# zhenyuw16/Uni3DETR

Measured on AMD Instinct MI355X. Metric: scenes/sec (fwd+bwd) SUN-RGB-D 20k pts, 300 queries, higher is better.
Workload: dtype bf16

## Files before the change

### include/u3d_hip.h

```cpp
#ifndef U3D_HIP_H_
#define U3D_HIP_H_

#include <stddef.h>
#include <stdint.h>

#ifdef __cplusplus
extern "C" {
#endif

typedef struct ihipStream_t* u3d_stream;

enum {
  U3D_OK = 0,
  U3D_ERR_ARG = -1,
  U3D_ERR_UNSUPPORTED = -2,
  U3D_ERR_LAUNCH = -3,
  U3D_ERR_WORKSPACE = -4
};

enum { U3D_F32 = 0, U3D_BF16 = 1 };

int32_t u3d_version(void);
const char* u3d_strerror(int32_t code);

// ... 244 lines not shown
                     int32_t* out_count, int32_t* out_off, void* workspace, int64_t workspace_bytes, u3d_stream s);

#define U3D_DET_TAIL_SOFT_NMS 3
#define U3D_DET_TAIL_MERGE 4
int64_t u3d_det_tail_pp_workspace(int32_t batch, int32_t nq, int32_t num_classes, int32_t max_num, int32_t box_dim, int32_t mode);
int32_t u3d_det_tail_pp(const float* prob, const float* fused, const float* boxes, int32_t batch, int32_t nq, int32_t num_classes,
                        int32_t box_dim, int32_t max_num, const float* center_range, float score_threshold, int32_t mode, float nms_thr,
                        const float* score_thr, int32_t num_thr, float soft_sigma, float soft_prune, float* out_boxes, float* out_scores,
                        int32_t* out_labels, int32_t* out_count, int32_t* out_off, void* workspace, int64_t workspace_bytes, u3d_stream s);

int32_t u3d_tap_gather_sum(const void* p, const int32_t* nbr, int32_t ld, const int32_t* n_dev, int32_t n_cap, int32_t c,
                           int32_t kvol, int32_t dtype, void* out, u3d_stream s);
int32_t u3d_tap_gather_sum_add(const void* p, const int32_t* nbr, int32_t ld, const int32_t* n_dev, int32_t n_cap, int32_t c,
                               int32_t kvol, int32_t dtype, const void* addend, void* out, u3d_stream s);

int32_t u3d_layernorm_blocks(int32_t n);
int32_t u3d_layernorm_fwd(const void* x, int32_t x_dtype, int32_t n, int32_t c, const float* gamma, const float* beta,
                          float eps, int32_t relu, void* y, int32_t y_dtype, float* mean, float* rstd, u3d_stream s);
int32_t u3d_layernorm_bwd(const void* dy, int32_t y_dtype, const void* x, int32_t x_dtype, int32_t n, int32_t c,
                          const float* gamma, const float* beta, const float* mean, const float* rstd, int32_t relu,
                          void* dx, float* partial, u3d_stream s);

int64_t u3d_det_loss_workspace(int32_t L, int32_t m);
int32_t u3d_det_loss_fwd(const float* cls, const float* box, const float* iou_logit, const float* tgt, const int64_t* lab,
                         const float* w, const float* iou_true, const float* cls_avg, const float* npos, const float* code_w,
                         int32_t L, int32_t m, int32_t c, int32_t code, int32_t tdim, float alpha, float w_cls, float w_box,
                         float w_iou, float eps, float* out, void* workspace, int64_t workspace_bytes, u3d_stream s);
int32_t u3d_det_loss_bwd(const float* cls, const float* box, const float* iou_logit, const float* tgt, const int64_t* lab,
                         const float* w, const float* iou_true, const float* cls_avg, const float* npos, const float* code_w,
                         const float* gout, int32_t L, int32_t m, int32_t c, int32_t code, int32_t tdim, float alpha, float w_cls,
// ... 262 lines not shown
```

### uni3detr_amd/csrc/glds_epilogue.inc

```
  f32x4 cs[WN], cq[WN];
#pragma unroll
  for (int b = 0; b < WN; ++b) { cs[b] = (f32x4){0.f, 0.f, 0.f, 0.f}; cq[b] = (f32x4){0.f, 0.f, 0.f, 0.f}; }
#pragma unroll
  for (int a = 0; a < WM; ++a) {
    const int m = m0 + (wm * WM + a) * 16 + li;
    if (m >= n_out) continue;
#pragma unroll
    for (int b = 0; b < WN; ++b) {
      const int col = col0 + (wn * WN + b) * 16 + 4 * g;
      if (col < cout) {
        f32x4 v = acc[a][b];
        if (bias) {
          if (GLDS_EPI_ADDEND && (relu & 2)) {
            if constexpr (F32OUT) v += *(const f32x4*)(bias + (long long)m * cout + col);
            else v += __builtin_convertvector(*(const bf16x4*)((const u16*)bias + (long long)m * cout + col), f32x4);
          } else { const f32x4 bv = *(const f32x4*)(bias + col); v += bv; }
        }
        if (relu & 1) { v[0] = fmaxf(v[0], 0.f); v[1] = fmaxf(v[1], 0.f); v[2] = fmaxf(v[2], 0.f); v[3] = fmaxf(v[3], 0.f); }
        if constexpr (F32OUT) {
          *(f32x4*)((float*)out + (long long)m * cout + col) = v;
          if (stats) { cs[b] += v; cq[b] += v * v; }
          continue;
        }
        const bf16x4 o = __builtin_convertvector(v, bf16x4);
        *(bf16x4*)(out + (long long)m * cout + col) = o;
        if (stats) {
          const f32x4 vr = __builtin_convertvector(o, f32x4);
          if (GLDS_EPI_ADDEND && bn.x) {
            constexpr int CPR = BN / 8, SWZ = (CPR - 1) & 15;
            const int row = (wm * WM + a) * 16 + li, cc = (wn * WN + b) * 2 + (g >> 1);
            *(bf16x4*)(smem + ((row * CPR + (cc ^ (row & SWZ))) * 8 + (g & 1) * 4)) = o;
          } else {
            cs[b] += vr;
            cq[b] += vr * vr;
          }
        }
      }
    }
  }
  if (GLDS_EPI_ADDEND && stats && bn.x) {
// ... 13 lines not shown
          red[(wm * 2 + 0) * BN + cl] = s1;
          red[(wm * 2 + 1) * BN + cl] = s2;
        }
      }
    __syncthreads();
    for (int t = tid; t < 2 * BN; t += NW * 64) {
      const int which = t / BN, cl = t % BN;
      if (col0 + cl < cout) {
        double a = 0.0;
#pragma unroll
        for (int k = 0; k < WAVES_M; ++k) a += (double)red[(k * 2 + which) * BN + cl];
        stats[((long long)tile * 2 + which) * cout + col0 + cl] = a;
      }
    }
  }
```

### uni3detr_amd/csrc/igemm_bf16.hip

```cpp
#include "igemm_common.h"
#include "conv_in.h"
#include "igemm_direct.h"

struct BnEpi {
  const u16* x = nullptr;
  const u16* y = nullptr;
  const float *mean = nullptr, *invstd = nullptr, *gamma = nullptr, *beta = nullptr;
  int relu = 0, pad = 0;
};
template <int BM, int BN, int NT>
__device__ __forceinline__ void bn_bwd_tile_sums(const BnEpi bn, u16* smem, int m0, int col0, int n_out, int cout, int tile,
                                              double* __restrict__ stats, int tid) {
  constexpr int CPR = BN / 8, SWZ = (CPR - 1) & 15, R = NT / CPR, ROWS = BM / R, BATCH = ROWS < 8 ? ROWS : (ROWS % 8 == 0 ? 8 : (ROWS % 6 == 0 ? 6 : 4));
  static_assert(NT % CPR == 0 && BM % R == 0 && ROWS % BATCH == 0, "tile / thread mismatch");
  const int cc = tid % CPR, r0 = tid / CPR;
  const int col = col0 + cc * 8;
  const bool from_y = bn.relu && bn.y, remask = bn.relu && !bn.y;
  float s0[8], s1[8], mu[8], is[8], ga[8], be[8];
#pragma unroll
  for (int e = 0; e < 8; ++e) { s0[e] = 0.f; s1[e] = 0.f; mu[e] = 0.f; is[e] = 0.f; ga[e] = 0.f; be[e] = 0.f; }
  __syncthreads();
  if (col < cout) {
#pragma unroll
    for (int e = 0; e < 8; ++e) { mu[e] = bn.mean[col + e]; is[e] = bn.invstd[col + e]; }
// ... 239 lines not shown
template <int WAVES_M, int WAVES_N, int WM, int WN, bool WK, int BK = 64>
static int launch_igemm_fwd(const void* in, const void* w, const int32_t* nbr, int ld, void* out, const int32_t* n_out_dev,
                            int n_out_cap, int cin, int cout, int kvol, hipStream_t s, const float* bias = nullptr, int relu = 0) {
  constexpr int BM = WAVES_M * WM * 16, BN = WAVES_N * WN * 16;
  constexpr int LDA = BK + 8, LDW = WK ? BN + 16 : BK + 8;
  const size_t lds = 2 * (size_t)(BM * LDA + (WK ? BK * LDW : BN * LDW)) * 2;
  auto kern = k_igemm_fwd<WAVES_M, WAVES_N, WM, WN, WK, BK>;
  if (lds > 64 * 1024) U3D_ALLOW_LDS(kern, lds);
  dim3 grid(u3d_cdiv(n_out_cap, BM), u3d_cdiv(cout, BN));
  hipLaunchKernelGGL(kern, grid, dim3(WAVES_M * WAVES_N * 64), lds, s, (const u16*)in, (const u16*)w, nbr, ld, (u16*)out, n_out_dev,
                     n_out_cap, cin, cout, kvol, bias, relu);
  return hipGetLastError() == hipSuccess ? U3D_OK : U3D_ERR_LAUNCH;
}


template <int WAVES_M, int WAVES_N, int WM, int WN, bool F32OUT = false>
__device__ __forceinline__ void igemm_glds_body(const u16* __restrict__ in, const u16* __restrict__ w, const int* __restrict__ nbr,
                                                int ld, u16* __restrict__ out, const int* __restrict__ n_out_dev, int n_out_cap,
                                                int cin, int cout, int kvol, const float* __restrict__ bias, int relu,
                                                double* __restrict__ stats, const BnEpi bn) {
  constexpr int NW = WAVES_M * WAVES_N;
  constexpr int BM = WAVES_M * WM * 16, BN = WAVES_N * WN * 16, BK = 64;
  constexpr int A_ELEMS = BM * BK, W_ELEMS = BN * BK;
  constexpr int STAGE_ELEMS = A_ELEMS + W_ELEMS;
  constexpr int SEGS_A = BM / 8 / NW, SEGS_W = BN / 8 / NW;
  static_assert(BM % (8 * NW) == 0 && BN % (8 * NW) == 0, "tile/wave mismatch");
  extern __shared__ __attribute__((aligned(16))) u16 smem[];

  const int n_out = min(*n_out_dev, n_out_cap);
  const int tile = u3d_xcd_tile(blockIdx.x, (n_out + BM - 1) / BM);
  if (tile < 0) return;
  const int m0 = tile * BM;
  const int col0 = blockIdx.y * BN;
  const int tid = threadIdx.x, lane = tid & 63;
  const int wv = __builtin_amdgcn_readfirstlane(tid >> 6);
  const int wm = wv / WAVES_N, wn = wv % WAVES_N;
  const int kchunks = cin / BK;
  const int nstage = kvol * kchunks;

  f32x4 acc[WM][WN];
#pragma unroll
  for (int a = 0; a < WM; ++a)
#pragma unroll
    for (int b = 0; b < WN; ++b) acc[a][b] = (f32x4){0.f, 0.f, 0.f, 0.f};

  const __amdgpu_buffer_rsrc_t in_rs = __builtin_amdgcn_make_buffer_rsrc((void*)in, 0, -1, 0x00020000);
  const __amdgpu_buffer_rsrc_t w_rs = __builtin_amdgcn_make_buffer_rsrc((void*)w, 0, -1, 0x00020000);
  const unsigned row_bytes = (unsigned)cin * 2u;
  const int lrow = lane >> 3, lslot = lane & 7;
  unsigned a_part16[SEGS_A], w_voff[SEGS_W];
  int arow[SEGS_A];
#pragma unroll
  for (int u = 0; u < SEGS_A; ++u) {
    const int r = (wv * SEGS_A + u) * 8 + lrow;
    arow[u] = r;
    a_part16[u] = (unsigned)(lslot ^ ((r >> 1) & 7)) * 16u;
  }
#pragma unroll
  for (int u = 0; u < SEGS_W; ++u) {
    const int r = (wv * SEGS_W + u) * 8 + lrow;
    const int part = lslot ^ ((r >> 1) & 7);
    w_voff[u] = (col0 + r < cout) ? (unsigned)((col0 + r) * cin + part * 8) * 2u : 0xFFFFFFFFu;
  }
  int idx_cur[SEGS_A], idx_nxt[SEGS_A];
  auto load_idx_next = [&](int stage) {
    const int kap = stage % kvol;
#pragma unroll
    for (int u = 0; u < SEGS_A; ++u) {
      int m = m0 + arow[u];
      int mc = m < n_out ? m : n_out - 1;
      idx_nxt[u] = nbr ? nbr[(long long)kap * ld + mc] : mc;
    }
  };
  auto advance_idx = [&]() {
#pragma unroll
    for (int u = 0; u < SEGS_A; ++u) idx_cur[u] = (m0 + arow[u] < n_out) ? idx_nxt[u] : -1;
  };
  auto issue = [&](int st, int buf) {
    const int kap = st % kvol, c0 = (st / kvol) * BK;
    u16* Ab = smem + buf * STAGE_ELEMS + wv * (SEGS_A * 512);
    u16* Wb = smem + buf * STAGE_ELEMS + A_ELEMS + wv * (SEGS_W * 512);
    const unsigned a_soff = (unsigned)c0 * 2u;
    const unsigned w_soff = (unsigned)(kap * cin * cout + c0) * 2u;
#pragma unroll
    for (int u = 0; u < SEGS_A; ++u) {
      unsigned voff = idx_cur[u] >= 0 ? (unsigned)idx_cur[u] * row_bytes + a_part16[u] : 0xFFFFFFFFu;
      __builtin_amdgcn_raw_ptr_buffer_load_lds(in_rs, (lds_void_ptr)(Ab + u * 512), 16, voff, a_soff, 0, 0);
    }
#pragma unroll
    for (int u = 0; u < SEGS_W; ++u)
      __builtin_amdgcn_raw_ptr_buffer_load_lds(w_rs, (lds_void_ptr)(Wb + u * 512), 16, w_voff[u], w_soff, 0, 0);
  };
#if GLDS_FRAG_B128
  auto issue_one = [&](int st, int buf, int q) {
    const int kap = st % kvol, c0 = (st / kvol) * BK;
    if (q < SEGS_A) {
      u16* Ab = smem + buf * STAGE_ELEMS + wv * (SEGS_A * 512);
      unsigned voff = idx_cur[q] >= 0 ? (unsigned)idx_cur[q] * row_bytes + a_part16[q] : 0xFFFFFFFFu;
      __builtin_amdgcn_raw_ptr_buffer_load_lds(in_rs, (lds_void_ptr)(Ab + q * 512), 16, voff, (unsigned)c0 * 2u, 0, 0);
    } else {
      const int u = q - SEGS_A;
      u16* Wb = smem + buf * STAGE_ELEMS + A_ELEMS + wv * (SEGS_W * 512);
      __builtin_amdgcn_raw_ptr_buffer_load_lds(w_rs, (lds_void_ptr)(Wb + u * 512), 16, w_voff[u], (unsigned)(kap * cin * cout + c0) * 2u, 0, 0);
    }
  };
  const int g = lane >> 4, li = lane & 15, fsw = (lane >> 1) & 7;
  int foff[2];
#pragma unroll
  for (int ks = 0; ks < 2; ++ks) foff[ks] = ((ks * 4 + g) ^ fsw) << 3;
  typedef const volatile s16x8 __attribute__((address_space(3))) * lds_vptr;
// ... 5 lines not shown
  const int g = lane >> 4, li = lane & 15, fsw = (lane >> 1) & 7;
  int foff[2][2];
#pragma unroll
  for (int ks = 0; ks < 2; ++ks)
#pragma unroll
    for (int j = 0; j < 2; ++j) foff[ks][j] = (((ks * 4 + (g >> 1) + 2 * j) ^ fsw) << 3) + (g & 1) * 4;
  typedef const volatile s16x4 __attribute__((address_space(3))) * lds_vptr;
  auto frag = [&](const u16* rowp, int ks) {
    s16x4 x = *(lds_vptr)(rowp + foff[ks][0]);
    s16x4 y = *(lds_vptr)(rowp + foff[ks][1]);
    s16x8 v = {x[0], x[1], x[2], x[3], y[0], y[1], y[2], y[3]};
    return __builtin_bit_cast(bf16x8, v);
  };

#endif
  load_idx_next(0);
  advance_idx();
  load_idx_next(1 < nstage ? 1 : 0);
  issue(0, 0);
  __syncthreads();
  for (int st = 0; st < nstage; ++st) {
    const int buf = st & 1;
    const int nx = st + 1 < nstage ? st + 1 : st;
    advance_idx();
    load_idx_next(st + 2 < nstage ? st + 2 : nstage - 1);
#if !GLDS_DMA_SPREAD
    issue(nx, buf ^ 1);
#endif
    const u16* A = smem + buf * STAGE_ELEMS + (wm * WM * 16 + li) * BK;
    const u16* W = smem + buf * STAGE_ELEMS + A_ELEMS + (wn * WN * 16 + li) * BK;
#pragma unroll
    for (int ks = 0; ks < 2; ++ks) {
      bf16x8 af[WM];
#pragma unroll
      for (int a = 0; a < WM; ++a) af[a] = frag(A + a * 16 * BK, ks);
#pragma unroll
      for (int b = 0; b < WN; ++b) {
        bf16x8 bfr = frag(W + b * 16 * BK, ks);
#pragma unroll
        for (int a = 0; a < WM; ++a) acc[a][b] = __builtin_amdgcn_mfma_f32_16x16x32_bf16(bfr, af[a], acc[a][b], 0, 0, 0);
#if GLDS_DMA_SPREAD
        {
          constexpr int NQ = SEGS_A + SEGS_W, NG = (GLDS_DMA_SPREAD == 1) ? 2 * WN : (GLDS_DMA_SPREAD == 3 ? (WN > 1 ? WN / 2 : 1) : (GLDS_DMA_SPREAD == 4 ? WN + WN / 2 : WN));
          constexpr int PER = (NQ + NG - 1) / NG;
          const int grp = ks * WN + b;
          if (grp < NG) {
#pragma unroll
            for (int j = 0; j < PER; ++j)
              if (grp * PER + j < NQ) issue_one(nx, buf ^ 1, grp * PER + j);
          }
          __builtin_amdgcn_sched_barrier(0);
        }
#endif
      }
    }
    __syncthreads();
  }
#define GLDS_EPI_ADDEND (BM != 256 || BN != 256)
#include "glds_epilogue.inc"
#undef GLDS_EPI_ADDEND
}

#ifndef GLDS8_PRIO
#define GLDS8_PRIO 1
#endif
#ifndef GLDS8_BALANCE
#define GLDS8_BALANCE 1
#endif
#ifndef GLDS8_STAGGER
#define GLDS8_STAGGER 1
#endif
template <bool F32OUT = false, int RB = 4>
__device__ __forceinline__ void igemm_glds8_body(const u16* __restrict__ in, const u16* __restrict__ w, const int* __restrict__ nbr,
                                                 int ld, u16* __restrict__ out, const int* __restrict__ n_out_dev, int n_out_cap,
// ... 432 lines not shown
U3D_GLDS_KERNEL_X(k_igemm_glds_256x256, GLDS256_CFG)
U3D_GLDS_KERNEL(k_igemm_glds_256x128, 4, 2, 4, 4)
U3D_GLDS_KERNEL(k_igemm_glds_128x64, 4, 1, 2, 4)
U3D_GLDS_KERNEL(k_igemm_glds_128x128, 2, 2, 4, 4)
#undef U3D_GLDS_KERNEL
#define U3D_GLDS_KERNEL_F32O(NAME, A, B, C, D)                                                                                   \
  __global__ __launch_bounds__(A* B * 64) void NAME(const u16* in, const u16* w, const int* nbr, int ld, u16* out,               \
                                                    const int* n_out_dev, int n_out_cap, int cin, int cout, int kvol,            \
                                                    const float* bias, int relu, double* stats, BnEpi bn) {                      \
    igemm_glds_body<A, B, C, D, true>(in, w, nbr, ld, out, n_out_dev, n_out_cap, cin, cout, kvol, bias, relu, stats, bn);         \
  }
U3D_GLDS_KERNEL_F32O(k_igemm_glds_128x64_f32o, 4, 1, 2, 4)
U3D_GLDS_KERNEL_F32O(k_igemm_glds_128x128_f32o, 2, 2, 4, 4)
#undef U3D_GLDS_KERNEL_F32O
typedef void (*glds_kernel_t)(const u16*, const u16*, const int*, int, u16*, const int*, int, int, int, int, const float*, int, double*, BnEpi);


struct GldsKernel {
  glds_kernel_t bf16, f32;
  int rows, cols, threads;
  size_t lds;
  bool addend;
};
#define GLDS_GEOM(A, B, C, D) A * C * 16, B * D * 16, A * B * 64, (size_t)2 * (A * C * 16 + B * D * 16) * 64 * 2
#define GLDS_GEOM_X(...) GLDS_GEOM(__VA_ARGS__)
enum { G_256x256, G8_256x256, G8_192x256, G8_256x128, G8_192x128, G_256x128, G_128x128, G_128x64, G_COUNT };
static const GldsKernel GLDS_KERNELS[G_COUNT] = {
    {k_igemm_glds_256x256, nullptr, GLDS_GEOM_X(GLDS256_CFG), false},
    {k_igemm_glds8_256x256, k_igemm_glds8_256x256_f32o, 256, 256, 512, 2 * (256 + 256) * 64 * 2, true},
    {k_igemm_glds8_192x256, k_igemm_glds8_192x256_f32o, 192, 256, 512, 2 * (256 + 256) * 64 * 2, true},
// ... 141 lines not shown
}

extern "C" int32_t u3d_igemm_dgrad_bnstats_bf16(const void* in, const void* w, const int32_t* nbr, int32_t ld, const void* addend, void* out,
                                                const int32_t* n_out_dev, int32_t n_out_cap, int32_t cin, int32_t cout, int32_t kvol,
                                                const u3d_bn_epi* bn, double* stats, u3d_stream s) {
  U3D_REQUIRE(in && w && out && n_out_dev && nbr && bn && bn->x && bn->mean && bn->invstd && stats, U3D_ERR_ARG);
  U3D_REQUIRE(!bn->relu || bn->y || (bn->gamma && bn->beta), U3D_ERR_ARG);
  const FwdPlan p = fwd_plan(n_out_cap, cin, cout, kvol, true, true, EPI_BN_BWD);
  if (!p.served()) return U3D_ERR_UNSUPPORTED;
  BnEpi e;
  e.x = (const u16*)bn->x; e.y = (const u16*)bn->y; e.mean = bn->mean; e.invstd = bn->invstd; e.gamma = bn->gamma; e.beta = bn->beta;
  e.relu = bn->relu;
  return fwd_launch(p, in, w, nbr, ld, out, n_out_dev, n_out_cap, cin, cout, kvol, s, addend, addend ? 2 : 0, stats, e);
}

extern "C" int32_t u3d_igemm_fwd_bf16(const void* in, const void* w, const int32_t* nbr, int32_t ld, void* out,
                                      const int32_t* n_out_dev, int32_t n_out_cap, int32_t cin, int32_t cout, int32_t kvol,
                                      int32_t transpose_w, u3d_stream s) {
  U3D_REQUIRE(in && w && out && n_out_dev && (nbr || kvol == 1), U3D_ERR_ARG);
  if (!transpose_w && convin_shape(cin, cout, kvol))
    return u3d_launch_conv_in_fwd(in, w, nbr, ld, out, n_out_dev, n_out_cap, kvol, s);
  const FwdPlan p = fwd_plan(n_out_cap, cin, cout, kvol, nbr != nullptr, transpose_w != 0, EPI_PLAIN);
  if (p.served()) return fwd_launch(p, in, w, nbr, ld, out, n_out_dev, n_out_cap, cin, cout, kvol, s);
  if (n_out_cap > 0 && cin % 16 == 0 && cout % 16 == 0 && cin <= 64 && cout <= 64 && (cin < 64 || cout < 64)) {
#define IG_SMALL(WNV, BKV)                                                                                                                          \
    return transpose_w ? launch_igemm_fwd<4, 1, IGEMM_SMALL_WM, WNV, false, BKV>(in, w, nbr, ld, out, n_out_dev, n_out_cap, cin, cout, kvol, s)   \
                       : launch_igemm_fwd<4, 1, IGEMM_SMALL_WM, WNV, true, BKV>(in, w, nbr, ld, out, n_out_dev, n_out_cap, cin, cout, kvol, s);
    if (cin == 16 || cin == 32) {
      if (cout == 16) { IG_SMALL(1, 32) }
      if (cout == 32) { IG_SMALL(2, 32) }
// ... 17 lines not shown
```

### uni3detr_amd/native.py

```python
import ctypes as C
import os

import numpy as np
import torch

from . import abi

_HERE = os.path.dirname(os.path.abspath(__file__))
LIB_PATH = os.environ.get("U3D_LIB_PATH") or os.path.join(_HERE, "libu3d_hip.so")

_ABI = abi.load()
_K = _ABI.constants


def _struct(c_name, py_name):
    return abi.structure(_ABI.structs[c_name], py_name)


def _slot_names(prefix):
    names = sorted((v, n[len(prefix):]) for n, v in _K.items() if n.startswith(prefix))
    assert [v for v, _ in names] == list(range(len(names))) and names[-1][1] == "COUNT" and _K[prefix + "COUNT"] == len(names) - 1
    return [n for _, n in names[:-1]]


# ... 1343 lines not shown
    n = len(counts)
    assert n == len(caps) and n <= 8 and flag.dtype == torch.float32
    _check(lib().u3d_capacity_flag(_ptr_array(counts), (C.c_int32 * max(n, 1))(*[int(c) for c in caps]), n, _ptr(flag), _stream()),
           "capacity_flag")


def tap_gather_sum(p, nbr, n_dev, n, c, kvol, addend=None):
    out = torch.empty((n, c), dtype=p.dtype, device=p.device)
    if addend is not None:
        assert addend.shape == out.shape and addend.dtype == out.dtype and addend.is_contiguous()
    _check(lib().u3d_tap_gather_sum_add(_ptr(p), _ptr(nbr), nbr.shape[1], _ptr(n_dev), n, c, kvol, dtype_code(p), _ptr(addend), _ptr(out),
                                        _stream()), "tap_gather_sum")
    return out


def _ptr_array(tensors):
    arr = (C.c_void_p * len(tensors))()
    for i, t in enumerate(tensors):
        arr[i] = t.data_ptr()
    return arr


def _batch_chunks(outs, maxb):
    o, n = 0, len(outs)
    while o < n:
        e = min(n, o + maxb)
        while e < n and e > o + 1 and outs[e].data_ptr() == outs[e - 1].data_ptr():
            e -= 1
        if e < n and outs[e].data_ptr() == outs[e - 1].data_ptr():
            raise U3DError("a group of batch slots with one output is larger than the batch limit")
# ... 646 lines not shown
```

### uni3detr_amd/plugin/dense.py

```python

import numpy as np
import torch
from torch import nn

from .. import native as nv
from .. import sparse as sp
from ..registry import BACKBONES, NECKS


def _conv(cfg, cin, cout, kernel, stride=1, padding=0):
    cfg = dict(cfg)
    t = cfg.pop("type")
    if t != "Conv3d":
        raise NotImplementedError("the HIP dense path implements the Conv3d variant used by every shipped config")
    if cfg.get("bias", True):
        raise NotImplementedError("shipped configs build these convolutions with bias=False")
    return nn.Conv3d(cin, cout, kernel, stride=stride, padding=padding, **cfg)


def _norm(cfg, c):
    cfg = dict(cfg)
    t = cfg.pop("type")
    assert t == "BN3d", "shipped configs use BN3d"
    cfg.pop("requires_grad", None)
# ... 9 lines not shown
    _cache = {}

    @classmethod
    def conv(cls, device, batch, dims_in, ksize, stride, pad):
        key = ("c", str(device), batch, tuple(dims_in), tuple(ksize), tuple(stride), tuple(pad))
        g = cls._cache.get(key)
        if g is None:
            dims_out = tuple((d + 2 * p - k) // s + 1 for d, k, s, p in zip(dims_in, ksize, stride, pad))
            n_in = batch * dims_in[0] * dims_in[1] * dims_in[2]
            n_out = batch * dims_out[0] * dims_out[1] * dims_out[2]
            one = all(k == 1 for k in ksize) and all(s == 1 for s in stride)
            fwd = None if one else nv.dense_nbr_table(batch, dims_out, dims_in, ksize, stride, pad, 0, device)
            bwd = None if one else nv.dense_nbr_table(batch, dims_in, dims_out, ksize, stride, pad, 1, device)
            n_in_dev = torch.tensor([n_in], dtype=torch.int32, device=device)
            n_out_dev = torch.tensor([n_out], dtype=torch.int32, device=device)
            g = (sp.ConvGeom(fwd, bwd, n_in, n_in_dev, n_out, n_out_dev, kind="dense", strided=any(s > 1 for s in stride)), dims_out)
            cls._cache[key] = g
        return g

    @classmethod
    def upsample_index(cls, device, batch, dims_in, s):
        key = ("u", str(device), batch, tuple(dims_in), s)
        v = cls._cache.get(key)
        if v is None:
            D, H, W = dims_in
            b = torch.arange(batch, device=device).view(-1, 1, 1, 1)
            z = torch.arange(D, device=device).view(1, -1, 1, 1)
            y = torch.arange(H * s, device=device).view(1, 1, -1, 1)
            x = torch.arange(W * s, device=device).view(1, 1, 1, -1)
            in_row = ((b * D + z) * H + y // s) * W + x // s
            tap = (y % s) * s + (x % s)
# ... 175 lines not shown
```

### uni3detr_amd/sparse.py

```python
import collections
import contextlib
import os

import torch

from . import native as nv
from .shadow import conv_weights, halo_packs

K3, S1, P1 = (3, 3, 3), (1, 1, 1), (1, 1, 1)


class Level:

    def __init__(self, grid, coords, n, n_dev):
        self.grid, self.coords, self.n, self.n_dev = grid, coords, n, n_dev
        self.dims, self.batch = grid.dims, grid.batch
        self._subm = None
        self._halo = None

    def halo(self):
        if self._halo is None:
            h = nv.SubmHalo(self.subm_tables()[0], self.n_dev, self.n) if self.n <= nv.SubmHalo.MAX_ROWS else None
            self._halo = h if (h is not None and h.ok) else False
        return self._halo or None
# ... 31 lines not shown
    def __init__(self, n):
        self.n = self.remaining = n
        self.acc = None

    def step(self, din):
        self.remaining -= 1
        if self.remaining > 0:
            self.acc = din
            return None
        self.acc, self.remaining = None, self.n
        return din


class ConvGeom:

    def __init__(self, nbr_fwd, nbr_bwd, n_in, n_in_dev, n_out, n_out_dev, kind="sparse", strided=False):
        self.strided = strided
        self.nbr_fwd, self.nbr_bwd = nbr_fwd, nbr_bwd
        self.n_in, self.n_in_dev, self.n_out, self.n_out_dev = n_in, n_in_dev, n_out, n_out_dev
        self.kind = kind
        self.level = None


def level_from_coors(coors, batch, dims):
    dev = coors.device
    g = nv.BitGrid(batch, dims, dev)
    g.mark(coors)
    g.scan()
    n = coors.shape[0]
    g.set_row_capacity(n)
    rank = g.rank(coors)
    lvl = Level(g, g.coords(n), n, g.count_dev)
    return lvl, rank


def subm_geom(lvl):
# ... 2 lines not shown
    g.level = lvl
    return g


def strided_level(lvl, ksize, stride, pad, capacity=None):
    dims_out = tuple((d + 2 * p - k) // s + 1 for d, k, s, p in zip(lvl.dims, ksize, stride, pad))
    g = nv.BitGrid(lvl.batch, dims_out, lvl.coords.device)
    g.mark_strided(lvl.coords, lvl.n_dev, ksize, stride, pad)
    g.scan()
    n_out = int(g.count_dev.item()) if capacity is None else int(capacity)
    if capacity is not None:
        g.set_row_capacity(n_out)
    out = Level(g, g.coords(n_out), n_out, g.count_dev)
    fwd = lvl.grid.nbr_table(out.coords, out.n_dev, ksize, stride, pad, 0)
    bwd = g.nbr_table(lvl.coords, lvl.n_dev, ksize, stride, pad, 1)
    return out, ConvGeom(fwd, bwd, lvl.n, lvl.n_dev, n_out, out.n_dev, strided=True)


REV_SUBM_TABLE = True
SUBM_HALO = os.environ.get("U3D_SUBM_HALO", "1") == "1"
HALO_WGRAD = True
HALO_128 = True
STRIDED_DGRAD_SPLIT = True
NMAJOR_FWD = True
STRIDED_SPLIT_MIN_RATIO = 16
STRIDED_SPLIT_SPARSE_RATIO = 16


_CONV_USES = {}


def reset_conv_uses():
    _CONV_USES.clear()
    _PLANES_BWD.clear()


SPLIT_BF16 = os.environ.get("U3D_SPLIT_BF16", "1") == "1"
SPLIT_FUSED_ADD = True
# ... 71 lines not shown
            t = torch.arange(n_rows, dtype=torch.int32, device=geom.n_out_dev.device).view(1, -1)
        elif isinstance(t, nv.RevNbr):
            t = t.t.flip(0)
        lo = torch.where(t >= 0, t + plane, t)
        cache[key] = torch.cat([t, lo] if which == "wgrad" else [t, t, lo], 0).contiguous()
    return cache[key]


def _halo_of(geom, kvol, cin, cout):
    if not (SUBM_HALO and REV_SUBM_TABLE and geom.level is not None and kvol == 27 and cin == cout
            and (cin == 64 or (cin == 128 and HALO_128)) and geom.n_out >= 4096):
        return None
    return geom.level.halo()


_ConvRoute = collections.namedtuple("_ConvRoute", "split nmajor halo kvol cin cout strided_split")


def _conv_route(feats, kio_shape, geom):
    kvol, cin, cout = kio_shape[0] * kio_shape[1] * kio_shape[2], kio_shape[3], kio_shape[4]
    bf16 = feats.dtype == torch.bfloat16
    nmajor = NMAJOR_FWD and bf16 and ((cin % 64 == 0 and cout % 64 == 0) or nv.direct_serves(cin, cout, kvol))
    split = _split_serves(feats, cin, cout, kvol)
    if split == "narrow" and geom.nbr_fwd is None:
        split = None
    halo = _halo_of(geom, kvol, cin, cout) if (nmajor and not split) else None
    strided_split = bool(STRIDED_DGRAD_SPLIT and geom.strided and kvol > 1 and (bf16 or split == "wide") and cout % 64 == 0
                         and (kvol * cin) % 64 == 0
                         and geom.n_out * (STRIDED_SPLIT_SPARSE_RATIO if geom.kind == "sparse" else STRIDED_SPLIT_MIN_RATIO) <= geom.n_in)
    return _ConvRoute(split, nmajor, halo, kvol, cin, cout, strided_split)


def _pending_addend(ctx):
    tok, fan = ctx.res_token, ctx.fan_token
    dres = tok.dres if tok is not None else None
    facc = fan.acc if fan is not None else None
    if dres is not None and facc is not None:
        return dres + facc
    return facc if dres is None else dres


def _finish_din(ctx, din, taken):
    tok, fan = ctx.res_token, ctx.fan_token
    if din is not None and not taken:
        if fan is not None and fan.acc is not None:
# ... 100 lines not shown

def _input_grad(ctx, r, wc, dout):
    g, kvol, cin, cout = ctx.geom, r.kvol, r.cin, r.cout
    nbr = g.nbr_bwd if kvol > 1 else None
    add = _pending_addend(ctx)
    fits = add is not None and add.dtype == dout.dtype and add.is_contiguous() and tuple(add.shape) == (g.n_in, cin)
    if r.strided_split:
        prod = nv.linear_bf16(dout, wc.view(kvol * cin, cout), None, False)
        fan = ctx.fan_token
        if not (fits and fan is not None and add is fan.acc):
            add = None
        return nv.tap_gather_sum(prod, nbr, g.n_in_dev, g.n_in, cin, kvol, addend=add), add is not None
    bt = ctx.bn_in
    if bt is not None and (bt.c != cin or not (add is None or fits)):
        bt = None
    if r.halo is not None:
        if cin != 64:
            bt = None
        if not fits:
            add = None
        pk = ctx.pk_bwd if ctx.pk_bwd is not None else nv.subm_halo_wpack(wc)
        din = nv.subm_halo_conv(dout, pk, r.halo, krev=True, addend=add, want_stats=bt is not None, tag="spconv_dgrad",
                                bn_epi=None if bt is None else bt.epi)
        if bt is not None:
            din, st, tr = din
            bt.partial = (st, tr)
        return din, add is not None
    res = nv.spconv_dgrad_bnstats(dout, wc, nbr, g.n_in_dev, g.n_in, cin, add, bt.epi) if (bt is not None and kvol > 1) else None
    if res is not None:
        bt.partial = (res[1], res[2])
# ... 220 lines not shown
```

Before: 424.4.

## Add stride-class sorted dgrad for strided sparse convs with per-tile tap masks

New measurement: 426.6, median of 6. Within noise of the previous version (+0.5%).

```diff
diff --git a/include/u3d_hip.h b/include/u3d_hip.h
--- a/include/u3d_hip.h
+++ b/include/u3d_hip.h
@@ -282,6 +282,16 @@
 int32_t u3d_tap_gather_sum_add(const void* p, const int32_t* nbr, int32_t ld, const int32_t* n_dev, int32_t n_cap, int32_t c,
                                int32_t kvol, int32_t dtype, const void* addend, void* out, u3d_stream s);
 
+int64_t u3d_stride_sort_workspace(int32_t n_cap);
+int32_t u3d_stride_sort(const int32_t* nbr, int32_t ld, const int32_t* n_dev, int32_t n_cap, const int32_t* coors,
+                        const int32_t dims[3], const int32_t ksize[3], const int32_t stride[3], const int32_t pad[3],
+                        int32_t tile_rows, int32_t* order, int32_t* tbl, int32_t tbl_ld, int32_t* tile_mask, void* workspace,
+                        int64_t workspace_bytes, u3d_stream s);
+int32_t u3d_igemm_dgrad_sorted_plan(int32_t n_cap, int32_t cin, int32_t cout, int32_t kvol, int32_t* rows, int32_t* cols);
+int32_t u3d_igemm_dgrad_sorted_bf16(const void* in, const void* w, const int32_t* tbl, int32_t ld, const int32_t* tile_mask,
+                                    const int32_t* order, const void* addend, void* out, const int32_t* n_dev, int32_t n_cap,
+                                    int32_t cin, int32_t cout, int32_t kvol, u3d_stream s);
+
 int32_t u3d_layernorm_blocks(int32_t n);
 int32_t u3d_layernorm_fwd(const void* x, int32_t x_dtype, int32_t n, int32_t c, const float* gamma, const float* beta,
                           float eps, int32_t relu, void* y, int32_t y_dtype, float* mean, float* rstd, u3d_stream s);
diff --git a/uni3detr_amd/csrc/glds_epilogue.inc b/uni3detr_amd/csrc/glds_epilogue.inc
--- a/uni3detr_amd/csrc/glds_epilogue.inc
+++ b/uni3detr_amd/csrc/glds_epilogue.inc
@@ -1,3 +1,7 @@
+#ifndef GLDS_EPI_ROW
+#define GLDS_EPI_ROW(m) (m)
+#define GLDS_EPI_ROW_DEFAULTED
+#endif
   f32x4 cs[WN], cq[WN];
 #pragma unroll
   for (int b = 0; b < WN; ++b) { cs[b] = (f32x4){0.f, 0.f, 0.f, 0.f}; cq[b] = (f32x4){0.f, 0.f, 0.f, 0.f}; }
@@ -5,6 +9,7 @@
   for (int a = 0; a < WM; ++a) {
     const int m = m0 + (wm * WM + a) * 16 + li;
     if (m >= n_out) continue;
+    const int mo = GLDS_EPI_ROW(m);
 #pragma unroll
     for (int b = 0; b < WN; ++b) {
       const int col = col0 + (wn * WN + b) * 16 + 4 * g;
@@ -12,18 +17,18 @@
         f32x4 v = acc[a][b];
         if (bias) {
           if (GLDS_EPI_ADDEND && (relu & 2)) {
-            if constexpr (F32OUT) v += *(const f32x4*)(bias + (long long)m * cout + col);
-            else v += __builtin_convertvector(*(const bf16x4*)((const u16*)bias + (long long)m * cout + col), f32x4);
+            if constexpr (F32OUT) v += *(const f32x4*)(bias + (long long)mo * cout + col);
+            else v += __builtin_convertvector(*(const bf16x4*)((const u16*)bias + (long long)mo * cout + col), f32x4);
           } else { const f32x4 bv = *(const f32x4*)(bias + col); v += bv; }
         }
         if (relu & 1) { v[0] = fmaxf(v[0], 0.f); v[1] = fmaxf(v[1], 0.f); v[2] = fmaxf(v[2], 0.f); v[3] = fmaxf(v[3], 0.f); }
         if constexpr (F32OUT) {
-          *(f32x4*)((float*)out + (long long)m * cout + col) = v;
+          *(f32x4*)((float*)out + (long long)mo * cout + col) = v;
           if (stats) { cs[b] += v; cq[b] += v * v; }
           continue;
         }
         const bf16x4 o = __builtin_convertvector(v, bf16x4);
-        *(bf16x4*)(out + (long long)m * cout + col) = o;
+        *(bf16x4*)(out + (long long)mo * cout + col) = o;
         if (stats) {
           const f32x4 vr = __builtin_convertvector(o, f32x4);
           if (GLDS_EPI_ADDEND && bn.x) {
@@ -67,3 +72,7 @@
       }
     }
   }
+#ifdef GLDS_EPI_ROW_DEFAULTED
+#undef GLDS_EPI_ROW
+#undef GLDS_EPI_ROW_DEFAULTED
+#endif
diff --git a/uni3detr_amd/csrc/igemm_bf16.hip b/uni3detr_amd/csrc/igemm_bf16.hip
--- a/uni3detr_amd/csrc/igemm_bf16.hip
+++ b/uni3detr_amd/csrc/igemm_bf16.hip
@@ -277,11 +277,13 @@
 }
 
 
-template <int WAVES_M, int WAVES_N, int WM, int WN, bool F32OUT = false>
+template <int WAVES_M, int WAVES_N, int WM, int WN, bool F32OUT = false, bool SORTED = false>
 __device__ __forceinline__ void igemm_glds_body(const u16* __restrict__ in, const u16* __restrict__ w, const int* __restrict__ nbr,
                                                 int ld, u16* __restrict__ out, const int* __restrict__ n_out_dev, int n_out_cap,
                                                 int cin, int cout, int kvol, const float* __restrict__ bias, int relu,
-                                                double* __restrict__ stats, const BnEpi bn) {
+                                                double* __restrict__ stats, const BnEpi bn,
+                                                const unsigned* __restrict__ tile_mask = nullptr,
+                                                const int* __restrict__ out_rows = nullptr) {
   constexpr int NW = WAVES_M * WAVES_N;
   constexpr int BM = WAVES_M * WM * 16, BN = WAVES_N * WN * 16, BK = 64;
   constexpr int A_ELEMS = BM * BK, W_ELEMS = BN * BK;
@@ -299,7 +301,24 @@
   const int wv = __builtin_amdgcn_readfirstlane(tid >> 6);
   const int wm = wv / WAVES_N, wn = wv % WAVES_N;
   const int kchunks = cin / BK;
-  const int nstage = kvol * kchunks;
+  unsigned sw_mask = 0, sw_rem = 0;
+  int sw_c = 0, sw_left = 0;
+  if constexpr (SORTED) {
+    sw_mask = __builtin_amdgcn_readfirstlane(tile_mask[tile]) & (kvol >= 32 ? 0xFFFFFFFFu : ((1u << kvol) - 1u));
+    sw_rem = sw_mask;
+    sw_left = __builtin_popcount(sw_mask) * kchunks;
+  }
+  const int nstage = SORTED ? sw_left : kvol * kchunks;
+  int sw_k1 = 0, sw_c1 = 0, sw_k2 = 0, sw_c2 = 0;
+  auto sw_next = [&](int& kap, int& c0) {
+    if (sw_left > 0) {
+      kap = __builtin_ctz(sw_rem);
+      c0 = sw_c;
+      sw_rem &= sw_rem - 1u;
+      if (sw_rem == 0u) { sw_rem = sw_mask; sw_c += BK; }
+      --sw_left;
+    }
+  };
 
   f32x4 acc[WM][WN];
 #pragma unroll
@@ -327,7 +346,7 @@
   }
   int idx_cur[SEGS_A], idx_nxt[SEGS_A];
   auto load_idx_next = [&](int stage) {
-    const int kap = stage % kvol;
+    const int kap = SORTED ? stage : stage % kvol;
 #pragma unroll
     for (int u = 0; u < SEGS_A; ++u) {
       int m = m0 + arow[u];
@@ -340,7 +359,7 @@
     for (int u = 0; u < SEGS_A; ++u) idx_cur[u] = (m0 + arow[u] < n_out) ? idx_nxt[u] : -1;
   };
   auto issue = [&](int st, int buf) {
-    const int kap = st % kvol, c0 = (st / kvol) * BK;
+    const int kap = SORTED ? sw_k1 : st % kvol, c0 = SORTED ? sw_c1 : (st / kvol) * BK;
     u16* Ab = smem + buf * STAGE_ELEMS + wv * (SEGS_A * 512);
     u16* Wb = smem + buf * STAGE_ELEMS + A_ELEMS + wv * (SEGS_W * 512);
     const unsigned a_soff = (unsigned)c0 * 2u;
@@ -356,7 +375,7 @@
   };
 #if GLDS_FRAG_B128
   auto issue_one = [&](int st, int buf, int q) {
-    const int kap = st % kvol, c0 = (st / kvol) * BK;
+    const int kap = SORTED ? sw_k1 : st % kvol, c0 = SORTED ? sw_c1 : (st / kvol) * BK;
     if (q < SEGS_A) {
       u16* Ab = smem + buf * STAGE_ELEMS + wv * (SEGS_A * 512);
       unsigned voff = idx_cur[q] >= 0 ? (unsigned)idx_cur[q] * row_bytes + a_part16[q] : 0xFFFFFFFFu;
@@ -392,16 +411,29 @@
   };
 
 #endif
+  if (!SORTED || nstage > 0) {
+  if constexpr (SORTED) {
+    sw_next(sw_k1, sw_c1);
+    load_idx_next(sw_k1);
+    advance_idx();
+    sw_k2 = sw_k1; sw_c2 = sw_c1;
+    sw_next(sw_k2, sw_c2);
+    load_idx_next(sw_k2);
+    issue(0, 0);
+    sw_k1 = sw_k2; sw_c1 = sw_c2;
+    sw_next(sw_k2, sw_c2);
+  } else {
   load_idx_next(0);
   advance_idx();
   load_idx_next(1 < nstage ? 1 : 0);
   issue(0, 0);
+  }
   __syncthreads();
   for (int st = 0; st < nstage; ++st) {
     const int buf = st & 1;
     const int nx = st + 1 < nstage ? st + 1 : st;
     advance_idx();
-    load_idx_next(st + 2 < nstage ? st + 2 : nstage - 1);
+    load_idx_next(SORTED ? sw_k2 : (st + 2 < nstage ? st + 2 : nstage - 1));
 #if !GLDS_DMA_SPREAD
     issue(nx, buf ^ 1);
 #endif
@@ -432,10 +464,17 @@
 #endif
       }
     }
+    if constexpr (SORTED) {
+      sw_k1 = sw_k2; sw_c1 = sw_c2;
+      sw_next(sw_k2, sw_c2);
+    }
     __syncthreads();
   }
-#define GLDS_EPI_ADDEND (BM != 256 || BN != 256)
+  }
+#define GLDS_EPI_ADDEND (SORTED || BM != 256 || BN != 256)
+#define GLDS_EPI_ROW(m) (SORTED ? out_rows[m] : (m))
 #include "glds_epilogue.inc"
+#undef GLDS_EPI_ROW
 #undef GLDS_EPI_ADDEND
 }
 
@@ -898,6 +937,23 @@
 U3D_GLDS_KERNEL_F32O(k_igemm_glds_128x128_f32o, 2, 2, 4, 4)
 #undef U3D_GLDS_KERNEL_F32O
 typedef void (*glds_kernel_t)(const u16*, const u16*, const int*, int, u16*, const int*, int, int, int, int, const float*, int, double*, BnEpi);
+
+#define U3D_GLDS_SORTED_KERNEL(NAME, A, B, C, D)                                                                                 \
+  __global__ __launch_bounds__(A* B * 64) void NAME(const u16* in, const u16* w, const int* tbl, int ld, u16* out,               \
+                                                    const int* n_out_dev, int n_out_cap, int cin, int cout, int kvol,            \
+                                                    const float* addend, int relu, const unsigned* tile_mask,                    \
+                                                    const int* out_rows) {                                                       \
+    igemm_glds_body<A, B, C, D, false, true>(in, w, tbl, ld, out, n_out_dev, n_out_cap, cin, cout, kvol, addend, relu, nullptr,   \
+                                             BnEpi{}, tile_mask, out_rows);                                                      \
+  }
+U3D_GLDS_SORTED_KERNEL(k_igemm_glds_sorted_128x64, 4, 1, 2, 4)
+U3D_GLDS_SORTED_KERNEL(k_igemm_glds_sorted_128x128, 2, 2, 4, 4)
+#define U3D_GLDS_SORTED_KERNEL_X(NAME, ...) U3D_GLDS_SORTED_KERNEL(NAME, __VA_ARGS__)
+U3D_GLDS_SORTED_KERNEL_X(k_igemm_glds_sorted_256x256, GLDS256_CFG)
+#undef U3D_GLDS_SORTED_KERNEL_X
+#undef U3D_GLDS_SORTED_KERNEL
+typedef void (*glds_sorted_kernel_t)(const u16*, const u16*, const int*, int, u16*, const int*, int, int, int, int, const float*, int,
+                                     const unsigned*, const int*);
 
 
 struct GldsKernel {
@@ -1069,6 +1125,42 @@
   return fwd_launch(p, in, w, nbr, ld, out, n_out_dev, n_out_cap, cin, cout, kvol, s, addend, addend ? 2 : 0, stats, e);
 }
 
+struct SortedPlan {
+  glds_sorted_kernel_t fn = nullptr;
+  int rows = 0, cols = 0, threads = 0;
+  size_t lds = 0;
+};
+static SortedPlan sorted_plan(int n_cap, int cin, int cout, int kvol) {
+  SortedPlan p;
+  if (n_cap <= 0 || cin <= 0 || cout <= 0 || cin % 64 != 0 || cout % 64 != 0 || kvol < 1 || kvol > 27) return p;
+  if (cout % 256 == 0 && (long long)u3d_cdiv(n_cap, 256) * (cout / 256) >= 128) {
+    p.fn = k_igemm_glds_sorted_256x256; p.rows = 256; p.cols = 256; p.threads = 512;
+  } else if (cout % 128 == 0) { p.fn = k_igemm_glds_sorted_128x128; p.rows = 128; p.cols = 128; p.threads = 256; }
+  else { p.fn = k_igemm_glds_sorted_128x64; p.rows = 128; p.cols = 64; p.threads = 256; }
+  p.lds = (size_t)2 * (p.rows + p.cols) * 64 * 2;
+  return p;
+}
+extern "C" int32_t u3d_igemm_dgrad_sorted_plan(int32_t n_cap, int32_t cin, int32_t cout, int32_t kvol, int32_t* rows, int32_t* cols) {
+  U3D_REQUIRE(rows && cols, U3D_ERR_ARG);
+  const SortedPlan p = sorted_plan(n_cap, cin, cout, kvol);
+  if (!p.fn) return U3D_ERR_UNSUPPORTED;
+  *rows = p.rows;
+  *cols = p.cols;
+  return U3D_OK;
+}
+extern "C" int32_t u3d_igemm_dgrad_sorted_bf16(const void* in, const void* w, const int32_t* tbl, int32_t ld, const int32_t* tile_mask,
+                                               const int32_t* order, const void* addend, void* out, const int32_t* n_dev, int32_t n_cap,
+                                               int32_t cin, int32_t cout, int32_t kvol, u3d_stream s) {
+  U3D_REQUIRE(in && w && tbl && tile_mask && order && out && n_dev && ld >= n_cap, U3D_ERR_ARG);
+  const SortedPlan p = sorted_plan(n_cap, cin, cout, kvol);
+  if (!p.fn) return U3D_ERR_UNSUPPORTED;
+  if (p.lds > 64 * 1024) U3D_ALLOW_LDS(p.fn, p.lds);
+  hipLaunchKernelGGL(p.fn, dim3(u3d_cdiv(n_cap, p.rows), cout / p.cols), dim3(p.threads), p.lds, (hipStream_t)s, (const u16*)in,
+                     (const u16*)w, tbl, ld, (u16*)out, n_dev, n_cap, cin, cout, kvol, (const float*)addend, addend ? 2 : 0,
+                     (const unsigned*)tile_mask, order);
+  return hipGetLastError() == hipSuccess ? U3D_OK : U3D_ERR_LAUNCH;
+}
+
 extern "C" int32_t u3d_igemm_fwd_bf16(const void* in, const void* w, const int32_t* nbr, int32_t ld, void* out,
                                       const int32_t* n_out_dev, int32_t n_out_cap, int32_t cin, int32_t cout, int32_t kvol,
                                       int32_t transpose_w, u3d_stream s) {
diff --git a/uni3detr_amd/csrc/stride_sort.hip b/uni3detr_amd/csrc/stride_sort.hip
--- /dev/null
+++ b/uni3detr_amd/csrc/stride_sort.hip
@@ -0,0 +1,154 @@
+#include "common.h"
+
+#define SSORT_MAX_CLASSES 64
+#define SSORT_BLOCK 256
+
+struct SortGeom {
+  int dz, dy, dx;
+  int s[3], p[3];
+  int ncls;
+};
+
+__device__ __forceinline__ int ssort_class(const int4* __restrict__ coors, const SortGeom& g, int m) {
+  int z, y, x;
+  if (coors) {
+    const int4 c = coors[m];
+    z = c.y; y = c.z; x = c.w;
+  } else {
+    x = m % g.dx;
+    const int t = m / g.dx;
+    y = t % g.dy;
+    z = (t / g.dy) % g.dz;
+  }
+  const int cz = (z + g.p[0]) % g.s[0], cy = (y + g.p[1]) % g.s[1], cx = (x + g.p[2]) % g.s[2];
+  return (cz * g.s[1] + cy) * g.s[2] + cx;
+}
+
+__device__ __forceinline__ int ssort_rank(int cls, int ncls, int (*cnt)[SSORT_BLOCK / 64], int& wave_rank) {
+  const int lane = threadIdx.x & 63, wv = threadIdx.x >> 6;
+  const unsigned long long below = (1ull << lane) - 1ull;
+  wave_rank = 0;
+  for (int c = 0; c < ncls; ++c) {
+    const unsigned long long b = __ballot(cls == c);
+    if (cls == c) wave_rank = __popcll(b & below);
+    if (lane == 0) cnt[c][wv] = __popcll(b);
+  }
+  __syncthreads();
+  return cls;
+}
+
+__global__ __launch_bounds__(SSORT_BLOCK) void k_ssort_hist(const int4* __restrict__ coors, SortGeom g, const int* __restrict__ n_dev,
+                                                           int n_cap, int nblocks, int* __restrict__ hist) {
+  __shared__ int cnt[SSORT_MAX_CLASSES][SSORT_BLOCK / 64];
+  const int n = min(*n_dev, n_cap);
+  const int m = blockIdx.x * SSORT_BLOCK + threadIdx.x;
+  const int cls = m < n ? ssort_class(coors, g, m) : -1;
+  int wr;
+  ssort_rank(cls, g.ncls, cnt, wr);
+  if ((int)threadIdx.x < g.ncls) {
+    int t = 0;
+#pragma unroll
+    for (int w = 0; w < SSORT_BLOCK / 64; ++w) t += cnt[threadIdx.x][w];
+    hist[threadIdx.x * nblocks + blockIdx.x] = t;
+  }
+}
+
+__global__ __launch_bounds__(1024) void k_ssort_scan(int* __restrict__ h, int e) {
+  __shared__ int part[1024];
+  const int tid = threadIdx.x, per = (e + 1023) / 1024;
+  const int b0 = min(tid * per, e), b1 = min(b0 + per, e);
+  int sum = 0;
+  for (int i = b0; i < b1; ++i) sum += h[i];
+  part[tid] = sum;
+  __syncthreads();
+  for (int off = 1; off < 1024; off <<= 1) {
+    const int v = tid >= off ? part[tid - off] : 0;
+    __syncthreads();
+    part[tid] += v;
+    __syncthreads();
+  }
+  int run = tid ? part[tid - 1] : 0;
+  for (int i = b0; i < b1; ++i) {
+    const int v = h[i];
+    h[i] = run;
+    run += v;
+  }
+}
+
+__global__ __launch_bounds__(SSORT_BLOCK) void k_ssort_scatter(const int4* __restrict__ coors, SortGeom g, const int* __restrict__ n_dev,
+                                                              int n_cap, int nblocks, const int* __restrict__ offs,
+                                                              int* __restrict__ order, const int* __restrict__ nbr, int ld, int kvol,
+                                                              int* __restrict__ tbl, int tld) {
+  __shared__ int cnt[SSORT_MAX_CLASSES][SSORT_BLOCK / 64];
+  const int n = min(*n_dev, n_cap);
+  const int m = blockIdx.x * SSORT_BLOCK + threadIdx.x;
+  const int cls = m < n ? ssort_class(coors, g, m) : -1;
+  int wr;
+  ssort_rank(cls, g.ncls, cnt, wr);
+  if (cls < 0) return;
+  const int wv = threadIdx.x >> 6;
+  int p = offs[cls * nblocks + blockIdx.x] + wr;
+  for (int w = 0; w < wv; ++w) p += cnt[cls][w];
+  if (p < 0 || p >= n_cap) return;
+  order[p] = m;
+  for (int k = 0; k < kvol; ++k) tbl[(long long)k * tld + p] = nbr[(long long)k * ld + m];
+}
+
+__global__ void k_ssort_mask(const int* __restrict__ n_dev, int n_cap, int kvol, int* __restrict__ tbl, int tld,
+                             unsigned* __restrict__ tile_mask) {
+  __shared__ unsigned wmask[16];
+  const int n = min(*n_dev, n_cap);
+  const int p = blockIdx.x * blockDim.x + threadIdx.x;
+  const bool live = p < n;
+  unsigned mask = 0;
+  for (int k = 0; k < kvol; ++k) {
+    int v = -1;
+    if (live) v = tbl[(long long)k * tld + p];
+    else if (p < tld) tbl[(long long)k * tld + p] = -1;
+    if (__ballot(v >= 0)) mask |= 1u << k;
+  }
+  if ((threadIdx.x & 63) == 0) wmask[threadIdx.x >> 6] = mask;
+  __syncthreads();
+  if (threadIdx.x == 0) {
+    unsigned t = 0;
+    for (int w = 0; w < (int)(blockDim.x >> 6); ++w) t |= wmask[w];
+    tile_mask[blockIdx.x] = t;
+  }
+}
+
+extern "C" int64_t u3d_stride_sort_workspace(int32_t n_cap) {
+  return (int64_t)SSORT_MAX_CLASSES * u3d_cdiv(n_cap > 0 ? n_cap : 1, SSORT_BLOCK) * (int64_t)sizeof(int32_t);
+}
+
+extern "C" int32_t u3d_stride_sort(const int32_t* nbr, int32_t ld, const int32_t* n_dev, int32_t n_cap, const int32_t* coors,
+                                   const int32_t dims[3], const int32_t ksize[3], const int32_t stride[3], const int32_t pad[3],
+                                   int32_t tile_rows, int32_t* order, int32_t* tbl, int32_t tbl_ld, int32_t* tile_mask, void* workspace,
+                                   int64_t workspace_bytes, u3d_stream s) {
+  U3D_REQUIRE(nbr && n_dev && dims && ksize && stride && pad && order && tbl && tile_mask && workspace, U3D_ERR_ARG);
+  U3D_REQUIRE(ld >= n_cap && tbl_ld >= n_cap && workspace_bytes >= u3d_stride_sort_workspace(n_cap), U3D_ERR_ARG);
+  U3D_REQUIRE(tile_rows >= 64 && tile_rows <= 1024 && tile_rows % 64 == 0, U3D_ERR_ARG);
+  SortGeom g;
+  long long kvol = 1, ncls = 1;
+  for (int d = 0; d < 3; ++d) {
+    U3D_REQUIRE(ksize[d] >= 1 && stride[d] >= 1 && pad[d] >= 0 && (coors || dims[d] >= 1), U3D_ERR_ARG);
+    g.s[d] = stride[d];
+    g.p[d] = pad[d];
+    kvol *= ksize[d];
+    ncls *= stride[d];
+  }
+  g.dz = dims[0]; g.dy = dims[1]; g.dx = dims[2];
+  if (kvol > 32 || ncls > SSORT_MAX_CLASSES) return U3D_ERR_UNSUPPORTED;
+  g.ncls = (int)ncls;
+  if (n_cap <= 0) return U3D_OK;
+  const int nblocks = u3d_cdiv(n_cap, SSORT_BLOCK);
+  int* hist = (int*)workspace;
+  hipStream_t st = (hipStream_t)s;
+  hipLaunchKernelGGL(k_ssort_hist, dim3(nblocks), dim3(SSORT_BLOCK), 0, st, (const int4*)coors, g, n_dev, n_cap, nblocks, hist);
+  hipLaunchKernelGGL(k_ssort_scan, dim3(1), dim3(1024), 0, st, hist, g.ncls * nblocks);
+  hipLaunchKernelGGL(k_ssort_scatter, dim3(nblocks), dim3(SSORT_BLOCK), 0, st, (const int4*)coors, g, n_dev, n_cap, nblocks, hist, order,
+                     nbr, ld, (int)kvol, tbl, tbl_ld);
+  hipLaunchKernelGGL(k_ssort_mask, dim3(u3d_cdiv(n_cap, tile_rows)), dim3(tile_rows), 0, st, n_dev, n_cap, (int)kvol, tbl, tbl_ld,
+                     (unsigned*)tile_mask);
+  U3D_CHECK_LAUNCH();
+  return U3D_OK;
+}
diff --git a/uni3detr_amd/native.py b/uni3detr_amd/native.py
--- a/uni3detr_amd/native.py
+++ b/uni3detr_amd/native.py
@@ -1381,6 +1381,56 @@
     return out
 
 
+def dgrad_sorted_plan(n, cin, cout, kvol):
+    r, c = C.c_int32(0), C.c_int32(0)
+    if lib().u3d_igemm_dgrad_sorted_plan(int(n), int(cin), int(cout), int(kvol), C.byref(r), C.byref(c)) != 0:
+        return None
+    return r.value, c.value
+
+
+class StrideSort:
+
+    def __init__(self, nbr, n_dev, n, coors, dims, ksize, stride, pad, tile_rows):
+        kvol, ld = nbr.shape
+        dev = nbr.device
+        self.n, self.tile_rows, self.nbr = int(n), int(tile_rows), nbr
+        self.order = torch.empty(max(self.n, 1), dtype=torch.int32, device=dev)
+        self.tbl = torch.empty((kvol, ld), dtype=torch.int32, device=dev)
+        self.tile_mask = torch.empty(max((self.n + tile_rows - 1) // tile_rows, 1), dtype=torch.int32, device=dev)
+        ws_bytes = int(lib().u3d_stride_sort_workspace(self.n))
+        ws = torch.empty(ws_bytes // 4, dtype=torch.int32, device=dev)
+        if coors is not None:
+            assert coors.dtype == torch.int32 and tuple(coors.shape) == (self.n, 4)
+        with torch.cuda.device(dev):
+            _check(lib().u3d_stride_sort(_ptr(nbr), ld, _ptr(n_dev), self.n, _ptr(coors), _I3(*dims), _I3(*ksize), _I3(*stride), _I3(*pad),
+                                         self.tile_rows, _ptr(self.order), _ptr(self.tbl), ld, _ptr(self.tile_mask), _ptr(ws), ws_bytes,
+                                         _stream()), "stride_sort")
+
+
+def stride_sort(nbr, n_dev, n, coors, dims, ksize, stride, pad, cin, cout):
+    plan = dgrad_sorted_plan(n, cin, cout, nbr.shape[0])
+    ncls = int(stride[0]) * int(stride[1]) * int(stride[2])
+    if plan is None or ncls > 64 or nbr.shape[0] != int(ksize[0]) * int(ksize[1]) * int(ksize[2]):
+        return None
+    return StrideSort(nbr, n_dev, n, coors, dims, ksize, stride, pad, plan[0])
+
+
+def spconv_dgrad_sorted(dout, w_nmajor, ss, n_dev, cout, addend=None):
+    kvol, cin = w_nmajor.shape[0], dout.shape[1]
+    plan = dgrad_sorted_plan(ss.n, cin, cout, kvol)
+    if plan is None or plan[0] != ss.tile_rows or dout.dtype != torch.bfloat16 or kvol != ss.tbl.shape[0]:
+        return None
+    out = torch.empty((ss.n, cout), dtype=dout.dtype, device=dout.device)
+    if addend is not None:
+        assert addend.shape == out.shape and addend.dtype == out.dtype and addend.is_contiguous()
+    region = timed_begin()
+    _check(lib().u3d_igemm_dgrad_sorted_bf16(_ptr(dout), _ptr(w_nmajor), _ptr(ss.tbl), ss.tbl.shape[1], _ptr(ss.tile_mask), _ptr(ss.order),
+                                             _ptr(addend), _ptr(out), _ptr(n_dev), ss.n, cin, cout, kvol, _stream()), "igemm_dgrad_sorted_bf16")
+    if region is not None:
+        timed_end(region, "spconv_dgrad", dout.shape[0], ss.n, cin, cout, kvol, ss.nbr, act_bytes=2, v2=True)
+    return out
+
+
 def _ptr_array(tensors):
     arr = (C.c_void_p * len(tensors))()
     for i, t in enumerate(tensors):
diff --git a/uni3detr_amd/plugin/dense.py b/uni3detr_amd/plugin/dense.py
--- a/uni3detr_amd/plugin/dense.py
+++ b/uni3detr_amd/plugin/dense.py
@@ -47,7 +47,9 @@
             bwd = None if one else nv.dense_nbr_table(batch, dims_in, dims_out, ksize, stride, pad, 1, device)
             n_in_dev = torch.tensor([n_in], dtype=torch.int32, device=device)
             n_out_dev = torch.tensor([n_out], dtype=torch.int32, device=device)
-            g = (sp.ConvGeom(fwd, bwd, n_in, n_in_dev, n_out, n_out_dev, kind="dense", strided=any(s > 1 for s in stride)), dims_out)
+            g = (sp.ConvGeom(fwd, bwd, n_in, n_in_dev, n_out, n_out_dev, kind="dense", strided=any(s > 1 for s in stride),
+                             sort_spec=None if all(s == 1 for s in stride) else (None, tuple(dims_in), tuple(ksize), tuple(stride), tuple(pad))),
+                 dims_out)
             cls._cache[key] = g
         return g
 
diff --git a/uni3detr_amd/sparse.py b/uni3detr_amd/sparse.py
--- a/uni3detr_amd/sparse.py
+++ b/uni3detr_amd/sparse.py
@@ -69,12 +69,25 @@
 
 class ConvGeom:
 
-    def __init__(self, nbr_fwd, nbr_bwd, n_in, n_in_dev, n_out, n_out_dev, kind="sparse", strided=False):
+    def __init__(self, nbr_fwd, nbr_bwd, n_in, n_in_dev, n_out, n_out_dev, kind="sparse", strided=False, sort_spec=None):
         self.strided = strided
+        self.sort_spec = sort_spec
+        self._sorted = {}
         self.nbr_fwd, self.nbr_bwd = nbr_fwd, nbr_bwd
         self.n_in, self.n_in_dev, self.n_out, self.n_out_dev = n_in, n_in_dev, n_out, n_out_dev
         self.kind = kind
         self.level = None
+
+    def stride_sort(self, cin, cout):
+        if self.sort_spec is None or self.nbr_bwd is None:
+            return None
+        plan = nv.dgrad_sorted_plan(self.n_in, cin, cout, self.nbr_bwd.shape[0])
+        if plan is None:
+            return None
+        if plan[0] not in self._sorted:
+            coors, dims, ksize, stride, pad = self.sort_spec
+            self._sorted[plan[0]] = nv.stride_sort(self.nbr_bwd, self.n_in_dev, self.n_in, coors, dims, ksize, stride, pad, cin, cout)
+        return self._sorted[plan[0]]
 
 
 def level_from_coors(coors, batch, dims):
@@ -107,7 +120,8 @@
     out = Level(g, g.coords(n_out), n_out, g.count_dev)
     fwd = lvl.grid.nbr_table(out.coords, out.n_dev, ksize, stride, pad, 0)
     bwd = g.nbr_table(lvl.coords, lvl.n_dev, ksize, stride, pad, 1)
-    return out, ConvGeom(fwd, bwd, lvl.n, lvl.n_dev, n_out, out.n_dev, strided=True)
+    return out, ConvGeom(fwd, bwd, lvl.n, lvl.n_dev, n_out, out.n_dev, strided=True,
+                         sort_spec=(lvl.coords, tuple(lvl.dims), tuple(ksize), tuple(stride), tuple(pad)))
 
 
 REV_SUBM_TABLE = True
@@ -115,6 +129,8 @@
 HALO_WGRAD = True
 HALO_128 = True
 STRIDED_DGRAD_SPLIT = True
+STRIDED_SORTED_OVER_SPLIT = False
+STRIDED_DGRAD_SORTED = os.environ.get("U3D_STRIDED_SORTED", "1") == "1"
 NMAJOR_FWD = True
 STRIDED_SPLIT_MIN_RATIO = 16
 STRIDED_SPLIT_SPARSE_RATIO = 16
@@ -216,7 +232,7 @@
     return geom.level.halo()
 
 
-_ConvRoute = collections.namedtuple("_ConvRoute", "split nmajor halo kvol cin cout strided_split")
+_ConvRoute = collections.namedtuple("_ConvRoute", "split nmajor halo kvol cin cout strided_split strided_sorted")
 
 
 def _conv_route(feats, kio_shape, geom):
@@ -230,7 +246,12 @@
     strided_split = bool(STRIDED_DGRAD_SPLIT and geom.strided and kvol > 1 and (bf16 or split == "wide") and cout % 64 == 0
                          and (kvol * cin) % 64 == 0
                          and geom.n_out * (STRIDED_SPLIT_SPARSE_RATIO if geom.kind == "sparse" else STRIDED_SPLIT_MIN_RATIO) <= geom.n_in)
-    return _ConvRoute(split, nmajor, halo, kvol, cin, cout, strided_split)
+    strided_sorted = bool(STRIDED_DGRAD_SORTED and geom.strided and kvol > 1 and bf16 and not split
+                          and (not strided_split or (STRIDED_SORTED_OVER_SPLIT and geom.kind == "dense"))
+                          and getattr(geom, "sort_spec", None) is not None and geom.nbr_bwd is not None
+                          and nv.dgrad_sorted_plan(geom.n_in, cout, cin, kvol) is not None)
+    strided_split = strided_split and not strided_sorted
+    return _ConvRoute(split, nmajor, halo, kvol, cin, cout, strided_split, strided_sorted)
 
 
 def _pending_addend(ctx):
@@ -361,6 +382,11 @@
     bt = ctx.bn_in
     if bt is not None and (bt.c != cin or not (add is None or fits)):
         bt = None
+    if r.strided_sorted and bt is None:
+        ss = g.stride_sort(cout, cin)
+        din = None if ss is None else nv.spconv_dgrad_sorted(dout, wc, ss, g.n_in_dev, cin, addend=add if fits else None)
+        if din is not None:
+            return din, bool(fits) or add is None
     if r.halo is not None:
         if cin != 64:
             bt = None
```
